# sakehl/SKA-SDP-Accelerate-gridding

Hardware: AMD Instinct MI355X
Metric: Mvis/s gridded (w-proj, 4096^2 grid) (higher is better)
Workload: dtype f64

## Files before the change

### ska-sdp-accelerate-gridding_amd/csrc/api.hip

```cpp

#include "common.h"
#include "imaging.h"

using namespace gridhip;

namespace {

int check_common(gridhip_ctx *ctx, int64_t H, int64_t Wd, const void *grid, int64_t n, const void *u,
                 const void *v, int64_t uv_stride)
{
    if (!ctx) return GRIDHIP_EINVAL;
    if (H <= 0 || Wd <= 0 || n < 0 || uv_stride < 1)
        return fail(ctx, GRIDHIP_EINVAL, "bad size (H=%lld Wd=%lld n=%lld uv_stride=%lld)", (long long)H,
                    (long long)Wd, (long long)n, (long long)uv_stride);
    if (!grid || (n > 0 && (!u || !v))) return fail(ctx, GRIDHIP_EINVAL, "null pointer");
    if (n > (int64_t)0x7fffff00) return fail(ctx, GRIDHIP_EUNSUPPORTED, "n must be < 2^31 per call");
    return GRIDHIP_OK;
}

int check_conv2(gridhip_ctx *ctx, int64_t H, int64_t Wd, const void *grid, int64_t n, const void *u, const void *v,
                int64_t uv_stride, const void *gcf, const void *vis, int64_t W, int64_t Q, int64_t gh, int64_t gw)
{
    GH_CHECK(check_common(ctx, H, Wd, grid, n, u, v, uv_stride));
    if (!gcf || (n > 0 && !vis)) return fail(ctx, GRIDHIP_EINVAL, "null pointer");
// ... 112 lines not shown
        }
    }
    if (rc == GRIDHIP_EUNSUPPORTED) {
        p->direct = true;
        return GRIDHIP_OK;
    }
    return rc;
}

int tile_kernels(gridhip_ctx *ctx, const Prep &p, const double *gcf, const double **out)
{
    ctx->last_path = p.direct ? 4 : !p.sorted ? 3 : p.g.P > 1 || p.g.fgh != p.g.gh || p.g.fgw != p.g.gw ? 2 : 1;
    ctx->last_geom[0] = p.g.ngroups;
    ctx->last_geom[1] = p.g.Tx;
    ctx->last_geom[2] = p.g.Ty;
    ctx->last_geom[3] = p.g.imoff > 0;
    *out = gcf;
    if (p.g.P == 1 && p.g.fgh == p.g.gh && p.g.fgw == p.g.gw) return GRIDHIP_OK;
    const int64_t nsl = (int64_t)p.g.W * p.g.Q * p.g.Q;
    const size_t elems = (size_t)nsl * p.g.P * p.g.gh * p.g.gw;
    GH_CHECK(ws_reserve(ctx, ctx->ktab, elems * 16));
    int blocks = (int)((elems + 255) / 256);
    if (blocks > ctx->num_cu * 16) blocks = ctx->num_cu * 16;
    hipLaunchKernelGGL(pad_kernels_kernel, dim3(blocks), dim3(256), 0, ctx->stream, p.g, nsl, (const double2 *)gcf,
                       (double2 *)ctx->ktab.ptr);
    GH_CHECK_HIP(ctx, hipGetLastError());
    *out = (const double *)ctx->ktab.ptr;
    return GRIDHIP_OK;
}

int tile_pass(gridhip_ctx *ctx, const Prep &p, const Geom &g, int64_t nrec, const double *table, const double *vis,
              const double *grid, bool degrid, bool may_keep)
{
    if (p.sorted)
        return launch_tile_grid_sorted(ctx, g, p.block, p.lds_sorted, p.nkeys, p.batch, nrec, table, vis,
                                       const_cast<double *>(grid), degrid, may_keep);
    if (degrid) return launch_tile_degrid(ctx, g, p.block, p.lds, nrec, table, grid, const_cast<double *>(vis));
    return launch_tile_grid(ctx, g, p.block, p.lds, nrec, table, vis, const_cast<double *>(grid));
}

}

extern "C" {

int gridhip_grid_dev(gridhip_ctx *ctx, int64_t H, int64_t Wd, double *grid, int64_t n, const double *u,
                     const double *v, int64_t uv_stride, const double *vis)
{
    GH_CHECK(check_common(ctx, H, Wd, grid, n, u, v, uv_stride));
    if (n > 0 && !vis) return fail(ctx, GRIDHIP_EINVAL, "null vis");
    GH_CHECK_HIP(ctx, hipSetDevice(ctx->device));
    mark(ctx, 0);
    mark(ctx, 1);
    GH_CHECK(launch_simple_grid(ctx, H, Wd, grid, n, u, v, uv_stride, vis));
    mark(ctx, 2);
    return GRIDHIP_OK;
}

int gridhip_convgrid2_dev(gridhip_ctx *ctx, int64_t H, int64_t Wd, double *grid, int64_t n, int64_t W, int64_t Q,
                          int64_t gh, int64_t gw, const double *gcf, const double *u, const double *v,
                          int64_t uv_stride, const int64_t *wbin, const double *vis)
{
    GH_CHECK(check_conv2(ctx, H, Wd, grid, n, u, v, uv_stride, gcf, vis, W, Q, gh, gw));
    GH_CHECK_HIP(ctx, hipSetDevice(ctx->device));
    Prep p;
    if (ctx->opt.variant == 1)
        p.direct = true;
// ... 122 lines not shown
```

### ska-sdp-accelerate-gridding_amd/csrc/common.h

```cpp
#pragma once
#include <hip/hip_runtime.h>
#include <stdint.h>
#include <stdio.h>
#include <string>
#include <unordered_set>
#include <utility>

#include "../../include/gridhip.h"

namespace gridhip {

struct VisRec {
    int32_t lxy;
    int32_t kslice;
    int32_t orig;
};
typedef unsigned long long RecWord;

struct Geom {
    int64_t H, Wd;
    int32_t W, Q, gh, gw;
    int32_t Tx, Ty;
    int32_t offx, offy;
    int32_t ntx, nty;
// ... 35 lines not shown
{
    return s < 0 ? x : __umulhi(x, m) >> s;
}
static inline void set_div_magic(Geom *g)
{
    div_magic(g->Tx, &g->mTx, &g->sTx);
    div_magic(g->Ty, &g->mTy, &g->sTy);
    div_magic(g->W, &g->mW, &g->sW);
    div_magic(g->P, &g->mP, &g->sP);
    div_magic(g->px, &g->mPx, &g->sPx);
}

static inline int bits_for(int64_t count)
{
    int b = 1;
    while (((int64_t)1 << b) < count) ++b;
    return b;
}
static inline void set_rec_bits(Geom *g)
{
    g->ob = bits_for(g->nvis);
    int64_t ks = g->nslices;
    if (g->per_vis && g->nvis > ks) ks = g->nvis;
    g->kb = bits_for(ks);
}
static inline bool rec_fits(const Geom &g, int limit = 64) { return g.ob + g.kb + 14 <= limit; }
__host__ __device__ __forceinline__ RecWord rec_pack(const Geom &g, int32_t lxy, int32_t kslice, int32_t orig)
{
    return (RecWord)(uint32_t)orig | (RecWord)(uint32_t)kslice << g.ob | (RecWord)((uint32_t)lxy & 0x7f) << (g.ob + g.kb) |
           (RecWord)(((uint32_t)lxy >> 16) & 0x7f) << (g.ob + g.kb + 7);
}

struct Options {
    int64_t tile = 0, block = 0, chunk = 0, wgroups = 0, variant = 0, sort = 0, dbg = 0, prepass = 0, fault_inject = 0, aw_cache = 1, aw_batch = 0, tile_x = 0, tile_y = 0, coarse_shift = 0, scatter_chunk = 0, count_unroll = 0, rec_bits = 0, wtable = 0, reserve_cus = 0, subfoot = 0, bigtile = 0, yield_cus = 0, bin_reuse = 0, list_reuse = 0;
};

struct Workspace {
    void *ptr = nullptr;
    size_t bytes = 0;
};

struct BinKey {
    Geom g;
    int64_t n, stride;
    const void *u, *v, *wbin;
    int64_t opt[5];
    const void *recs, *tables, *dig;
    uint64_t gen;
};
struct BinKeep {
    bool valid = false;
    BinKey key;
    bool pending = false;
    int backoff = 0;
    int32_t *host_flag = nullptr;
    int32_t *host_flag_dev = nullptr;
    int64_t verified = 0;
    bool verifying = false;
};
struct ListKeep {
    bool valid = false;
    uint64_t gen = 0;
    int64_t nrec = 0;
    int32_t nkeys = 0, batch = 0, ngroups = 0, ntiles = 0, Tx = 0, Ty = 0, ldw = 0, Q = 0, W = 0, P = 0;
    const void *list = nullptr, *staged = nullptr;
};
constexpr int SC_MATCH = 104, SC_VDROPPED = 105, SC_REUSED = 106, SC_GEN = 108;

struct ImagingState;

}

struct gridhip_ctx {
    int device = 0;
    hipStream_t own_stream = nullptr;
    hipStream_t stream = nullptr;
    hipEvent_t order_ev = nullptr;
    std::string err;
    gridhip::Options opt;
    gridhip::Workspace recs;
    gridhip::Workspace tables;
    gridhip::Workspace sorted;
    gridhip::Workspace recs_raw;
    gridhip::Workspace list_staged;
    gridhip::Workspace bin_digest;
    gridhip::Workspace recs_tmp;
    gridhip::Workspace blockhist;
    gridhip::Workspace ktab;
    gridhip::Workspace aw;
    int32_t *d_scalars = nullptr;
    uint64_t bin_gen = 0;
    gridhip::BinKeep keep;
    gridhip::ListKeep lists;
    int list_hold = 0;
    int64_t lists_reused = 0;
    int num_cu = 256;
    int max_lds = 160 * 1024;
    bool timing = false;
    static constexpr int EV_RING = 64;
    hipEvent_t ev[EV_RING * 3] = {};
    int64_t ev_calls = 0;
    bool ev_open = false;
    uint32_t attr_mask = 0;
    std::unordered_set<const void *> lds_raised;
    gridhip::ImagingState *img = nullptr;
    int last_path = 0;
    int last_geom[4] = {0, 0, 0, 0};
    int64_t aw_tables_built = 0;
};

namespace gridhip {

int fail(gridhip_ctx *ctx, int code, const char *fmt, ...);

#define GH_CHECK_HIP(ctx, call)                                                          \
    do {                                                                                 \
        hipError_t e__ = (call);                                                         \
        if (e__ != hipSuccess)                                                           \
            return gridhip::fail((ctx), e__ == hipErrorOutOfMemory ? GRIDHIP_ENOMEM      \
                                                                   : GRIDHIP_EHIP,       \
                                 "%s failed: %s (%s:%d)", #call, hipGetErrorString(e__), \
                                 __FILE__, __LINE__);                                    \
    } while (0)

#define GH_CHECK(expr)              \
    do {                            \
        int rc__ = (expr);          \
        if (rc__ != GRIDHIP_OK)     \
// ... 110 lines not shown
```

### ska-sdp-accelerate-gridding_amd/csrc/ctx.hip

```cpp
#include <stdarg.h>
#include <string.h>

#include <stdlib.h>

#include "common.h"
#include "imaging.h"

namespace gridhip {

int fail(gridhip_ctx *ctx, int code, const char *fmt, ...)
{
    char buf[512];
    va_list ap;
    va_start(ap, fmt);
    vsnprintf(buf, sizeof buf, fmt, ap);
    va_end(ap);
    if (ctx) ctx->err = buf;
    return code;
}

int ws_reserve(gridhip_ctx *ctx, Workspace &ws, size_t bytes)
{
    if (bytes <= ws.bytes) return GRIDHIP_OK;
    GH_CHECK_HIP(ctx, hipDeviceSynchronize());
// ... 412 lines not shown
    GH_CHECK_HIP(ctx, hipSetDevice(ctx->device));
    GH_CHECK_HIP(ctx, hipStreamSynchronize(ctx->stream));
    return GRIDHIP_OK;
}

static int64_t *opt_slot(gridhip_ctx *ctx, const char *key)
{
    if (!strcmp(key, "tile")) return &ctx->opt.tile;
    if (!strcmp(key, "tile_x")) return &ctx->opt.tile_x;
    if (!strcmp(key, "tile_y")) return &ctx->opt.tile_y;
    if (!strcmp(key, "block")) return &ctx->opt.block;
    if (!strcmp(key, "chunk")) return &ctx->opt.chunk;
    if (!strcmp(key, "wgroups")) return &ctx->opt.wgroups;
    if (!strcmp(key, "variant")) return &ctx->opt.variant;
    if (!strcmp(key, "sort")) return &ctx->opt.sort;
#ifdef GRIDHIP_TUNING
    if (!strcmp(key, "dbg")) return &ctx->opt.dbg;
#endif
    if (!strcmp(key, "prepass")) return &ctx->opt.prepass;
    if (!strcmp(key, "fault_inject")) return &ctx->opt.fault_inject;
    if (!strcmp(key, "aw_cache")) return &ctx->opt.aw_cache;
    if (!strcmp(key, "aw_batch")) return &ctx->opt.aw_batch;
    if (!strcmp(key, "coarse_shift")) return &ctx->opt.coarse_shift;
    if (!strcmp(key, "scatter_chunk")) return &ctx->opt.scatter_chunk;
    if (!strcmp(key, "count_unroll")) return &ctx->opt.count_unroll;
    if (!strcmp(key, "rec_bits")) return &ctx->opt.rec_bits;
    if (!strcmp(key, "wtable")) return &ctx->opt.wtable;
    if (!strcmp(key, "reserve_cus")) return &ctx->opt.reserve_cus;
    if (!strcmp(key, "subfoot")) return &ctx->opt.subfoot;
    if (!strcmp(key, "bigtile")) return &ctx->opt.bigtile;
    if (!strcmp(key, "yield_cus")) return &ctx->opt.yield_cus;
    if (!strcmp(key, "bin_reuse")) return &ctx->opt.bin_reuse;
    if (!strcmp(key, "list_reuse")) return &ctx->opt.list_reuse;
    if (!strcmp(key, "noise_bits")) return &ctx->img->noise_bits;
    if (!strcmp(key, "dft_slices")) return &ctx->img->dft_slices;
    if (!strcmp(key, "mosaic_cull")) return &ctx->img->mosaic_cull;
    if (!strcmp(key, "rm_stage")) return &ctx->img->rm_stage;
    return nullptr;
}

int gridhip_set_option(gridhip_ctx *ctx, const char *key, int64_t value)
{
    if (!ctx || !key) return GRIDHIP_EINVAL;
    int64_t *s = opt_slot(ctx, key);
    if (!s) return fail(ctx, GRIDHIP_EINVAL, "unknown option '%s'", key);
    if (value < 0 && s != &ctx->opt.aw_batch) return fail(ctx, GRIDHIP_EINVAL, "option '%s' must be >= 0", key);
    *s = value;
    return GRIDHIP_OK;
}

int gridhip_get_option(gridhip_ctx *ctx, const char *key, int64_t *value)
{
    if (!ctx || !key || !value) return GRIDHIP_EINVAL;
    if (!strcmp(key, "errors")) {
        GH_CHECK_HIP(ctx, hipSetDevice(ctx->device));
        int32_t h = 0;
        GH_CHECK_HIP(ctx, hipMemcpyAsync(&h, ctx->d_scalars + 2, sizeof h, hipMemcpyDeviceToHost, ctx->stream));
        GH_CHECK_HIP(ctx, hipStreamSynchronize(ctx->stream));
        *value = h;
        return GRIDHIP_OK;
    }
    {
        static const char *const names[4] = {"last_wgroups", "last_tile_x", "last_tile_y", "last_bigtile"};
        for (int i = 0; i < 4; ++i)
            if (!strcmp(key, names[i])) {
                *value = ctx->last_geom[i];
                return GRIDHIP_OK;
            }
    }
    if (!strcmp(key, "aw_tables_built")) {
        *value = ctx->aw_tables_built;
        return GRIDHIP_OK;
    }
    if (!strcmp(key, "prepass_verified")) {
        *value = ctx->keep.verified;
        return GRIDHIP_OK;
    }
    if (!strcmp(key, "prepass_reused")) {
        GH_CHECK_HIP(ctx, hipSetDevice(ctx->device));
        int32_t h = 0;
        GH_CHECK_HIP(ctx, hipMemcpyAsync(&h, ctx->d_scalars + SC_REUSED, sizeof h, hipMemcpyDeviceToHost, ctx->stream));
        GH_CHECK_HIP(ctx, hipStreamSynchronize(ctx->stream));
        *value = h;
        return GRIDHIP_OK;
    }
    if (!strcmp(key, "lists_reused")) {
        *value = ctx->lists_reused;
        return GRIDHIP_OK;
    }
    if (!strcmp(key, "last_path")) {
        *value = ctx->last_path;
        return GRIDHIP_OK;
    }
    if (!strcmp(key, "clock_khz") || !strcmp(key, "aw_clock_khz")) {
        GH_CHECK_HIP(ctx, hipSetDevice(ctx->device));
        int64_t h[4] = {0, 0, 0, 0};
        GH_CHECK_HIP(ctx, hipMemcpyAsync(h, ctx->d_scalars + (key[0] == 'a' ? 96 : 20), sizeof h, hipMemcpyDeviceToHost, ctx->stream));
        GH_CHECK_HIP(ctx, hipStreamSynchronize(ctx->stream));
        const int64_t cyc = h[2] - h[0], ticks = h[3] - h[1];
        *value = ticks > 0 && cyc > 0 ? (int64_t)((double)cyc / (double)ticks * 1e5) : 0;
        return GRIDHIP_OK;
    }
    if (!strncmp(key, "prof", 4) && key[4] >= '0' && key[4] <= '9') {
        const int slot = atoi(key + 4);
        if (slot < 0 || slot >= 32) return fail(ctx, GRIDHIP_EINVAL, "unknown option '%s'", key);
        GH_CHECK_HIP(ctx, hipSetDevice(ctx->device));
        int64_t h = 0;
        GH_CHECK_HIP(ctx, hipMemcpyAsync(&h, ctx->d_scalars + 32 + 2 * slot, sizeof h, hipMemcpyDeviceToHost,
                                         ctx->stream));
        GH_CHECK_HIP(ctx, hipStreamSynchronize(ctx->stream));
        *value = h;
        return GRIDHIP_OK;
    }
    int64_t *s = opt_slot(ctx, key);
    if (!s) return fail(ctx, GRIDHIP_EINVAL, "unknown option '%s'", key);
    *value = *s;
    return GRIDHIP_OK;
}

int gridhip_malloc(gridhip_ctx *ctx, void **dptr, int64_t bytes)
// ... 90 lines not shown
```

### ska-sdp-accelerate-gridding_amd/csrc/tile_sorted.hip

```cpp
#include "tile_common.h"

namespace gridhip {

__device__ __forceinline__ double readlane_f64(double x, int l)
{
    return __hiloint2double(__builtin_amdgcn_readlane(__double2hiint(x), l),
                            __builtin_amdgcn_readlane(__double2loint(x), l));
}

constexpr int SORTED_IM_OFF = 65528;

__device__ const int cut15[3][16] = {{0, 106, 211, 317, 422, 500, 578, 655, 733, 781, 829, 877, 926, 958, 991, 1024},
                                     {0, 108, 221, 329, 434, 513, 596, 677, 754, 800, 852, 898, 943, 969, 998, 1024},
                                     {0, 100, 202, 303, 401, 480, 562, 641, 718, 769, 824, 875, 925, 957, 992, 1024}};

struct SortedItem {
    int32_t valid, tile, grp, staged;
    int32_t v_lo;
};


template <int S, bool DEGRID, int ABL = 0, bool AW = false, bool BT = false>
__global__ void __launch_bounds__(1024, 4) tile_grid_sorted_kernel(Geom g, const RecWord *__restrict__ recs,
                                                                const int32_t *__restrict__ bin_start,
                                                                const int32_t *__restrict__ work_start,
                                                                const double2 *__restrict__ gcf,
                                                                double2 *__restrict__ vis,
                                                                double *__restrict__ grid, int nkeys, int batch,
                                                                int32_t *__restrict__ scalars,
                                                                double2 *__restrict__ sorted_vals,
                                                                uint2 *__restrict__ sorted_mo,
                                                                uint2 *__restrict__ keep_list,
                                                                int32_t *__restrict__ keep_staged, int istride,
                                                                int lists_valid)
{
    extern __shared__ double lds[];
    constexpr int S2 = S * S;
    constexpr int TAIL0 = S2 - ((S2 + 63) / 64 - 1) * 64;
    constexpr int EXTRA = DEGRID ? 0 : (TAIL0 > 32 && TAIL0 <= 34) ? TAIL0 - 32 : (S2 > 256 && TAIL0 <= 2) ? TAIL0 : 0;
    constexpr int S2E = S2 - EXTRA;
    constexpr int NSTEP_ALL = (S2E + 63) / 64;
    constexpr int TAIL = S2E - (NSTEP_ALL - 1) * 64;
    constexpr int MAXST = DEGRID ? 4 : 5;
    constexpr int FP = (NSTEP_ALL + MAXST - 1) / MAXST;
    constexpr int KST = (NSTEP_ALL + FP - 1) / FP;
    constexpr int REM = NSTEP_ALL % FP;
    constexpr int PBASE = NSTEP_ALL / FP;
    constexpr int NSTEP = KST;
    constexpr int LASTS = (REM == 0 ? KST : KST - 1) - 1;
    constexpr bool PAIR = !DEGRID && TAIL == 32;
    const int tid = threadIdx.x, nthr = blockDim.x;
    const int lane = tid & 63, wave = __builtin_amdgcn_readfirstlane(tid >> 6), nw = nthr >> 6;
    const int plane = g.lrows * g.ldw;
    const int IMO = BT ? g.imoff / 8 : SORTED_IM_OFF / 8;
    double *lre = lds, *lim = lds + IMO;
    int32_t *hist = reinterpret_cast<int32_t *>(lim + plane);
    const int hist_words = (nkeys + 1 + 3) & ~3;
    SortedItem *desc = reinterpret_cast<SortedItem *>(hist + hist_words);
    double2 *svals_wg = sorted_vals + (size_t)blockIdx.x * 2 * batch;
    uint2 *smo_wg = sorted_mo + (size_t)blockIdx.x * 2 * batch;
    int32_t *sorig_wg = reinterpret_cast<int32_t *>(sorted_vals) + (size_t)blockIdx.x * 2 * batch;

    constexpr bool STAGE_VALS = !DEGRID && AW;
    constexpr bool STAGE_ORIG = DEGRID && AW;
    const bool keeping = !AW && keep_list != nullptr;
    const bool kept = keeping && lists_valid && __builtin_amdgcn_readfirstlane(scalars[SC_MATCH]) == 1;
    const int maxcell = (g.Ty - 1) * g.ldw + g.Tx - 1;
    const bool solo = nw == 1;
    const bool is_sorter = wave == nw - 1;
    if (is_sorter && !solo && !(g.dbg & 512)) __builtin_amdgcn_s_setprio(3);
    const bool is_walker = solo || !is_sorter;
    const int nwalk = solo ? 1 : nw - 1;
    const int ncell = g.lrows * g.lcols;

    if (blockIdx.x == 0 && tid == 0) {
        long long *st = reinterpret_cast<long long *>(scalars + 20);
        st[0] = (long long)__builtin_amdgcn_s_memtime();
        st[1] = (long long)__builtin_amdgcn_s_memrealtime();
    }
    long long prof[7] = {0, 0, 0, 0, 0, 0, 0}, pt = 0;
#define GH_STAMP(i_)                        \
    if ((ABL & 16) && lane == 0) {          \
        const long long now_ = clock64();   \
        prof[i_] += now_ - pt;              \
        pt = now_;                          \
    }
    if ((ABL & 16) && lane == 0) pt = clock64();

    int32_t *queue = scalars + 4;
    int turn = 0;
    int items_left = ((int)blockIdx.x >= g.npersist) ? g.budget : 0x7fffffff;
    auto prepare = [&](int slot) {
        WorkItem w;
        int grp = 0, item = 0;
        bool have = false;
        if (items_left <= 0) turn = g.ngroups;
        --items_left;
        while (turn < g.ngroups) {
            grp = (blockIdx.x + turn) % g.ngroups;
            item = 0;
            if (lane == 0) item = atomicAdd(&queue[grp], 1);
            item = __builtin_amdgcn_readfirstlane(item);
            if (find_work_at(g, bin_start, work_start, grp, item, &w)) {
                have = true;
                break;
            }
            ++turn;
        }
        if (!have) {
            if (lane == 0) desc[slot].valid = 0;
            return;
        }
        GH_STAMP(0)
        const int first_plane = (grp * g.W + g.ngroups - 1) / g.ngroups;
        const int first_slice = first_plane * g.Q * g.Q * g.P;
        double2 *svals = svals_wg + (size_t)slot * batch;
        uint2 *smo = smo_wg + (size_t)slot * batch;
        int32_t *sorig = sorig_wg + (size_t)slot * batch;
        const int b_lo = w.v_lo;
        const int cnt = min(batch, w.v_hi - b_lo);
        int32_t *my_staged = keeping ? keep_staged + ((size_t)grp * istride + min(item, istride - 1)) : nullptr;
        if (kept) {
            if (lane == 0) {
                SortedItem d;
                d.valid = 1;
                d.tile = w.tile;
                d.grp = grp;
                d.staged = min(max(*my_staged, 0), max(cnt, 0));
                d.v_lo = b_lo;
                desc[slot] = d;
            }
            return;
        }
        if (keeping) smo = keep_list + b_lo;
        for (int i = lane; i <= nkeys; i += 64) hist[i] = 0;
        __builtin_amdgcn_fence(__ATOMIC_ACQ_REL, "wavefront");
        __builtin_amdgcn_wave_barrier();
        for (int r0 = lane; r0 < cnt; r0 += 8 * 64) {
            int key[8];
#pragma unroll
            for (int q = 0; q < 8; ++q) {
                bool off;
                key[q] = load_rec(recs, b_lo + min(r0 + q * 64, cnt - 1), g, &off).kslice - first_slice;
                if (AW) key[q] = (int)((unsigned)key[q] % (unsigned)nkeys);
                if (off) key[q] = -1;
            }
#pragma unroll
            for (int q = 0; q < 8; ++q)
                if (r0 + q * 64 < cnt && (unsigned)key[q] < (unsigned)nkeys) atomicAdd(&hist[key[q]], 1);
        }
        __builtin_amdgcn_fence(__ATOMIC_ACQ_REL, "wavefront");
        __builtin_amdgcn_wave_barrier();
        GH_STAMP(1)
        {
            const int per = (nkeys + 63) / 64;
            const int lo = min(lane * per, nkeys), hi = min(lo + per, nkeys);
            int sum = 0;
            for (int i = lo; i < hi; ++i) sum += hist[i];
            int incl = sum;
#pragma unroll
            for (int off = 1; off < 64; off <<= 1) {
                const int t = __shfl_up(incl, off, 64);
                if (lane >= off) incl += t;
            }
// ... 10 lines not shown
        int bad = 0;
        for (int r0 = lane; r0 < cnt; r0 += 8 * 64) {
            VisRec rec[8];
            double2 val[8];
            bool off[8];
#pragma unroll
            for (int q = 0; q < 8; ++q) rec[q] = load_rec(recs, b_lo + min(r0 + q * 64, cnt - 1), g, &off[q]);
            if (STAGE_VALS) {
#pragma unroll
                for (int q = 0; q < 8; ++q) val[q] = (ABL & 8) ? make_double2(1.0, (double)q) : load_nt(vis + rec[q].orig);
            }
#pragma unroll
            for (int q = 0; q < 8; ++q) {
                if (r0 + q * 64 >= cnt) break;
                int key = rec[q].kslice - first_slice;
                if (AW) key = (int)((unsigned)key % (unsigned)nkeys);
                if (off[q] || (unsigned)key >= (unsigned)nkeys) {
                    ++bad;
                    continue;
                }
                const int pos = atomicAdd(&hist[key], 1);
                if ((unsigned)pos < (unsigned)cnt) {
                    smo[pos] = make_uint2(((uint32_t)key << 16) | (uint32_t)((rec[q].lxy >> 16) * g.ldw + (rec[q].lxy & 0xffff)),
                                          (uint32_t)(AW ? rec[q].kslice : rec[q].orig));
                    if (STAGE_VALS) svals[pos] = val[q];
                    if (STAGE_ORIG) sorig[pos] = rec[q].orig;
                } else
                    ++bad;
            }
        }
        if (bad) atomicAdd(&scalars[2], bad);
        __builtin_amdgcn_fence(__ATOMIC_ACQ_REL, "wavefront");
        __builtin_amdgcn_wave_barrier();
        if (lane == 0) {
            SortedItem d;
            d.valid = 1;
            d.tile = w.tile;
            d.grp = grp;
            d.staged = min(hist[nkeys - 1], max(cnt, 0));
            d.v_lo = b_lo;
            desc[slot] = d;
            if (keeping) *my_staged = d.staged;
        }
        GH_STAMP(3)
    };

    int loff[NSTEP];
    const bool tail_ok = lane < TAIL || TAIL == 64;
#pragma unroll
    for (int s = 0; s < NSTEP; ++s) {
        int t = s * 64 + lane;
        if (FP == 1 && s == NSTEP - 1 && !tail_ok) t = PAIR ? s * 64 + lane - 32 : 0;
        loff[s] = (t / S) * g.ldw + (t % S);
    }
    const int ttail = tail_ok ? LASTS * 64 + lane : PAIR ? LASTS * 64 + lane - 32 : 0;
    const int lrow = lane / S, lcol = lane - lrow * S;

    auto walk = [&](int slot, int staged, int first_slice, int v_lo) {
        const double2 *svals = svals_wg + (size_t)slot * batch;
        const uint2 *smo = keeping ? keep_list + v_lo : smo_wg + (size_t)slot * batch;
        const int32_t *sorig = sorig_wg + (size_t)slot * batch;
        int seg_lo, seg_hi;
        if (nwalk == 15 && !DEGRID && !(g.dbg & 256)) {
            seg_lo = (int)(((int64_t)staged * cut15[g.dense][wave]) >> 10);
            seg_hi = (int)(((int64_t)staged * cut15[g.dense][wave + 1]) >> 10);
        } else {
            seg_lo = (int)(((int64_t)staged * wave) / nwalk);
            seg_hi = (int)(((int64_t)staged * (wave + 1)) / nwalk);
        }
        if (seg_lo >= seg_hi) return;
        auto load_list = [&](int b0, uint2 &mo, double2 &v, int32_t &o) {
            const int idx = max(min(b0 + lane, seg_hi - 1), seg_lo);
            mo = smo[idx];
            if (keeping) {
                const uint32_t cell = min(mo.x & 0xffffu, (uint32_t)maxcell), o_ = min(mo.y, (uint32_t)(g.nvis - 1));
                if (cell != (mo.x & 0xffffu) || o_ != mo.y) atomicAdd(&scalars[2], 1);
                mo.x = (mo.x & 0xffff0000u) | cell;
                mo.y = o_;
            }
            if (STAGE_VALS) v = svals[idx];
            if (STAGE_ORIG) o = sorig[idx];
        };
        auto load_value = [&](const uint2 &mo, double2 &v) {
            if (!DEGRID && !STAGE_VALS) v = (ABL & 8) ? make_double2(1.0, 2.0) : load_nt(vis + mo.y);
        };
        auto part_step0 = [&](int part) { return FP == 1 ? 0 : part * PBASE + min(part, REM); };
        auto part_nst = [&](int part) { return (FP == 1 || REM == 0 || part < REM) ? KST : KST - 1; };
        auto issue = [&](double2(&k)[NSTEP], int key, int len, int part) {
            key = min(max(key, 0), (AW ? g.nslices : nkeys) - 1);
            asm volatile("" : "+s"(key));
            const double2 *kp = gcf + (size_t)(first_slice + key) * S2 + 64 * part_step0(part);
            if (ABL & 4) {
#pragma unroll
                for (int s = 0; s < NSTEP; ++s) k[s] = make_double2((double)key, (double)(lane + s));
                return;
            }
            const int lofs = len > 0 ? lane : 0, lt = len > 0 ? ttail : 0;
            if (FP == 1) {
#pragma unroll
                for (int s = 0; s < NSTEP - 1; ++s) k[s] = kp[s * 64 + lofs];
                k[NSTEP - 1] = kp[lt];
            } else {
                const bool lastp = part == FP - 1, shortp = part_nst(part) < KST;
#pragma unroll
                for (int s = 0; s < NSTEP; ++s) {
                    int idx = s * 64 + lofs;
                    if (s == LASTS && lastp) idx = lt;
                    if (s == KST - 1 && shortp) idx = 0;
                    k[s] = kp[idx];
                }
            }
        };
        uint2 moN, moNN;
        double2 vN = make_double2(0.0, 0.0), vNN = make_double2(0.0, 0.0);
        int32_t oN = 0, oNN = 0;
        load_list(seg_lo, moN, vN, oN);
        load_list(seg_lo + 64, moNN, vNN, oNN);
        load_value(moN, vN);
        for (int b0 = seg_lo; b0 < seg_hi; b0 += 64) {
            const uint2 mo = moN;
            const double2 vB = vN;
            const int32_t oB = oN;
            moN = moNN;
            vN = vNN;
            oN = oNN;
            load_value(moN, vN);
            load_list(b0 + 128, moNN, vNN, oNN);
            const int bcnt = min(64, seg_hi - b0);
            const uint32_t mykey = AW ? mo.y : mo.x >> 16;
            const uint32_t prevkey = (uint32_t)__shfl_up((int)mykey, 1, 64);
            unsigned long long bits = __ballot(lane < bcnt && (lane == 0 || mykey != prevkey));
            double2 kx[EXTRA > 0 ? EXTRA : 1];
            if (EXTRA > 0) {
                const double2 *kp = gcf + (size_t)(first_slice + min((int)mykey, (AW ? g.nslices : nkeys) - 1)) * S2 + (S2 - EXTRA);
#pragma unroll
                for (int e = 0; e < EXTRA; ++e) kx[e] = (ABL & 4) ? make_double2(1.0, 2.0) : kp[e];
            }
            int lastKey = 0;
            int curKey = 0, curStart = 0, curLen = 0, curPart = FP - 1;
            auto advance = [&](int &key, int &start, int &len, int &part) {
                if (FP > 1 && curLen > 0 && curPart < FP - 1) {
                    ++curPart;
                    key = curKey;
                    start = curStart;
                    len = curLen;
                    part = curPart;
                    return;
                }
                if (bits == 0) {
                    key = lastKey;
                    start = 0;
// ... 147 lines not shown
                        const int row = lane >> 4;
                        if ((lane & 15) == 15 && i + row < len) {
                            const int32_t o = row == 0 ? oo[0] : row == 1 ? oo[1] : row == 2 ? oo[2] : oo[3];
                            if (g.P == 1 && FP == 1)
                                __builtin_nontemporal_store(dvec2_t{rr, ri}, reinterpret_cast<dvec2_t *>(vis + o));
                            else {
                                double *dst = reinterpret_cast<double *>(vis + o);
                                unsafeAtomicAdd(dst, rr);
                                unsafeAtomicAdd(dst + 1, ri);
                            }
                        }
                    }
                }
            };

            constexpr int NSETS = 3;
            double2 kS[NSETS][NSTEP];
            int keyS[NSETS], startS[NSETS], lenS[NSETS], partS[NSETS] = {0, 0, 0};
            static_assert(NSETS == 3, "initialiser of partS");
#pragma unroll
            for (int r = 0; r < NSETS - 1; ++r) {
                advance(keyS[r], startS[r], lenS[r], partS[r]);
                issue(kS[r], keyS[r], lenS[r], partS[r]);
            }
            int done = 0;
            for (;;) {
#pragma unroll
                for (int r = 0; r < NSETS; ++r) {
                    const int nx = (r + NSETS - 1) % NSETS;
                    advance(keyS[nx], startS[nx], lenS[nx], partS[nx]);
                    issue(kS[nx], keyS[nx], lenS[nx], partS[nx]);
                    asm volatile("" ::: "memory");
                    __builtin_amdgcn_sched_barrier(0);
                    process(kS[r], startS[r], lenS[r], partS[r]);
                    __builtin_amdgcn_sched_barrier(0);
                    if (FP == 1 || partS[r] == FP - 1) done += lenS[r];
                }
                if (done >= bcnt) break;
            }
            if (done > bcnt) {
#pragma unroll
                for (int r = 0; r < NSETS - 1; ++r) asm volatile("" ::"v"(kS[r][0].x), "v"(kS[r][NSTEP - 1].y));
            }
            if (EXTRA > 0 && !(ABL & 1) && lane < bcnt) {
                const int lb = (int)(mo.x & 0xffff);
#pragma unroll
                for (int e = 0; e < EXTRA; ++e) {
                    const int t = S2 - EXTRA + e;
                    double *cell = lre + (lb + (t / S) * g.ldw + (t % S));
                    __hip_atomic_fetch_add(cell, vB.x * kx[e].x - vB.y * kx[e].y, __ATOMIC_RELAXED,
                                           __HIP_MEMORY_SCOPE_WORKGROUP);
                    __hip_atomic_fetch_add(cell + IMO, vB.x * kx[e].y + vB.y * kx[e].x, __ATOMIC_RELAXED,
                                           __HIP_MEMORY_SCOPE_WORKGROUP);
                }
            }
        }
    };

    const int fl_r0 = (tid >> 1) / g.lcols, fl_c0 = (tid >> 1) - fl_r0 * g.lcols;
    const int fl_dr = (nthr >> 1) / g.lcols, fl_dc = (nthr >> 1) - fl_dr * g.lcols;

    if (is_sorter) prepare(0);
    if (!DEGRID) {
        for (int i = tid; i < plane; i += nthr) {
            lre[i] = 0.0;
            lim[i] = 0.0;
        }
    }
    __syncthreads();
    for (int cur = 0;; cur ^= 1) {
        const SortedItem d = desc[cur];
        if (!d.valid) break;
        const int first_plane = (d.grp * g.W + g.ngroups - 1) / g.ngroups;
        const int first_slice = first_plane * g.Q * g.Q * g.P;
        const int tx = d.tile % g.ntx, ty = d.tile / g.ntx;
        const int64_t ox = (int64_t)tx * g.Tx - g.offx, oy = (int64_t)ty * g.Ty - g.offy;
        if (DEGRID) {
            const double2 *gsrc = reinterpret_cast<const double2 *>(grid);
            for (int c = tid; c < ncell; c += nthr) {
                const int r_ = c / g.lcols, c_ = c - r_ * g.lcols;
                const int64_t gx = ox + c_, gy = oy + r_;
                double2 v = make_double2(0.0, 0.0);
                if (gx >= 0 && gy >= 0 && gx < g.Wd && gy < g.H) v = gsrc[gy * g.Wd + gx];
                lre[r_ * g.ldw + c_] = v.x;
                lim[r_ * g.ldw + c_] = v.y;
            }
            __syncthreads();
        }
        const long long walk_t0 = (ABL & 16) ? clock64() : 0;
        if (is_sorter && !solo) prepare(cur ^ 1);
        if (is_walker) {
            if ((ABL & 16) && wave == 0 && lane == 0) pt = clock64();
            walk(cur, d.staged, first_slice, d.v_lo);
            if ((ABL & 16) && wave == 0) GH_STAMP(4)
        }
        if (solo) prepare(cur ^ 1);
        if ((ABL & 16) && lane == 0)
            atomicAdd(reinterpret_cast<unsigned long long *>(scalars + 32) + 8 + wave, (unsigned long long)(clock64() - walk_t0));
        __syncthreads();
        if ((ABL & 16) && wave == 0) GH_STAMP(5)
        if (DEGRID) continue;

        {
            const int comp = tid & 1;
            int r_ = fl_r0, c_ = fl_c0;
            for (int e = tid; e < 2 * ncell; e += nthr) {
                const int64_t gx = ox + c_, gy = oy + r_;
                double *cell = (comp ? lim : lre) + r_ * g.ldw + c_;
                c_ += fl_dc;
                r_ += fl_dr;
                if (c_ >= g.lcols) {
                    c_ -= g.lcols;
                    ++r_;
                }
                const double val = *cell;
                if (val == 0.0) continue;
                *cell = 0.0;
                if ((ABL & 2) || gx < 0 || gy < 0 || gx >= g.Wd || gy >= g.H) continue;
                unsafeAtomicAdd(grid + 2 * (gy * g.Wd + gx) + comp, val);
            }
        }
        __syncthreads();
        if ((ABL & 16) && wave == 0) GH_STAMP(6)
    }
    if (blockIdx.x == 0 && tid == 0) {
        long long *st = reinterpret_cast<long long *>(scalars + 20);
        st[2] = (long long)__builtin_amdgcn_s_memtime();
        st[3] = (long long)__builtin_amdgcn_s_memrealtime();
    }
    if ((ABL & 16) && lane == 0 && (wave == 0 || (is_sorter && !solo))) {
        unsigned long long *out = reinterpret_cast<unsigned long long *>(scalars + 32);
        for (int i = 0; i < 7; ++i)
            if (prof[i]) atomicAdd(&out[i], (unsigned long long)prof[i]);
    }
#undef GH_STAMP
}

bool sorted_plan(const gridhip_ctx *ctx, const Geom &g, int block, int *nkeys, int *batch, size_t *lds_bytes)
{
    if (g.gh != g.gw || g.gh < 5 || g.gh > (g.per_vis ? 16 : 32)) return false;
    const int planes = (g.W + g.ngroups - 1) / g.ngroups + 1;
    const int64_t keys = g.per_vis ? 4096 : (int64_t)planes * g.Q * g.Q * g.P;
    if (keys >= 65536) return false;
    const size_t plane = (size_t)g.lrows * g.ldw * 8;
    if (plane > (size_t)(g.imoff > 0 ? g.imoff : SORTED_IM_OFF)) return false;
    const size_t tile = (size_t)(g.imoff > 0 ? g.imoff : SORTED_IM_OFF) + plane;
    const size_t hist = (size_t)((keys + 1 + 3) & ~3) * 4;
    if (tile + hist + 128 > (size_t)ctx->max_lds) return false;
    (void)block;
    int c = ctx->opt.chunk ? (int)ctx->opt.chunk : 16384;
    c = c < 64 ? 64 : c > 16384 ? 16384 : c;
    *nkeys = (int)keys;
    *batch = c;
    *lds_bytes = tile + hist + 128;
    return true;
}

int launch_tile_grid_sorted(gridhip_ctx *ctx, const Geom &g_in, int block, size_t lds_bytes, int nkeys, int batch,
                            int64_t n, const double *gcf, const double *vis, double *grid, bool degrid, bool may_keep)
{
    Geom g = g_in;
    Tables t = tables_of(ctx, g);
    const RecWord *recs = (const RecWord *)ctx->recs.ptr;
    if (g.chunk > batch) return fail(ctx, GRIDHIP_EINVAL, "sorted kernel: chunk %d exceeds its work-item capacity %d", g.chunk, batch);
    if (g.per_vis && g.imoff > 0) return fail(ctx, GRIDHIP_EUNSUPPORTED, "no big-tile form of the aw tile kernel");
    int per_cu = (int)((size_t)ctx->max_lds / lds_bytes);
    per_cu = per_cu < 1 ? 1 : per_cu > 4 ? 4 : per_cu;
    if (per_cu * block > 2048) per_cu = 2048 / block > 0 ? 2048 / block : 1;
    int cus = ctx->num_cu - (int)ctx->opt.reserve_cus;
    if (cus < g.ngroups) cus = g.ngroups;
    int nblk = cus * per_cu;
    nblk = ctx->opt.reserve_cus ? (nblk / g.ngroups) * g.ngroups : ((nblk + g.ngroups - 1) / g.ngroups) * g.ngroups;
    const int most = work_blocks(g, n);
    if (nblk > most) nblk = most > g.ngroups ? (most / g.ngroups) * g.ngroups : g.ngroups;
    g.npersist = nblk;
    g.budget = 0;
    if (ctx->opt.yield_cus > 0 && !ctx->opt.reserve_cus) {
        int k = (((int)ctx->opt.yield_cus + 31) / 32) * 32 * per_cu;
        k = (k / g.ngroups) * g.ngroups;
        if (k > 0 && nblk - k >= g.ngroups) {
            g.npersist = nblk - k;
            g.budget = 8;
            int extra = most - g.npersist;
            extra = extra > 2048 ? 2048 : extra;
            extra = (extra / g.ngroups) * g.ngroups;
            nblk = g.npersist + (extra > k ? extra : k);
        }
    }
    const dim3 gr(nblk), bl(block);
    const BinKeep &bk = ctx->keep;
    const bool keeping = may_keep && !g.per_vis && ctx->list_hold == 0 && ctx->opt.list_reuse != 1 && ctx->opt.bin_reuse != 1 && bk.valid &&
                         bk.key.gen == ctx->bin_gen && bk.key.recs == ctx->recs.ptr && bk.key.n == n && n > 0 &&
                         ctx->recs_raw.bytes >= (size_t)n * sizeof(uint2);
    const int istride = g.nrec / g.chunk + g.ntiles + 1;
    uint2 *klist = nullptr;
    int32_t *kstaged = nullptr;
    int lists_valid = 0;
    const ListKeep was = ctx->lists;
    ListKeep now;
    ctx->lists.valid = false;
    if (keeping) {
        GH_CHECK(ws_reserve(ctx, ctx->list_staged, (size_t)g.ngroups * istride * sizeof(int32_t)));
        klist = (uint2 *)ctx->recs_raw.ptr;
        kstaged = (int32_t *)ctx->list_staged.ptr;
        now.valid = true;
        now.gen = ctx->bin_gen;
        now.nrec = n;
        now.nkeys = nkeys, now.batch = batch, now.ngroups = g.ngroups, now.ntiles = g.ntiles;
        now.Tx = g.Tx, now.Ty = g.Ty, now.ldw = g.ldw, now.Q = g.Q, now.W = g.W, now.P = g.P;
        now.list = klist, now.staged = kstaged;
        lists_valid = bk.verifying && was.valid && was.gen + 1 == now.gen && was.nrec == now.nrec && was.nkeys == now.nkeys &&
                      was.batch == now.batch && was.ngroups == now.ngroups && was.ntiles == now.ntiles && was.Tx == now.Tx &&
                      was.Ty == now.Ty && was.ldw == now.ldw && was.Q == now.Q && was.W == now.W && was.P == now.P &&
                      was.list == now.list && was.staged == now.staged;
        if (lists_valid) ++ctx->lists_reused;
    }
    auto done = [&]() {
        ctx->lists = now;
        return GRIDHIP_OK;
    };
    const size_t nlist = (size_t)nblk * 2 * batch, nvals = g.per_vis ? nlist : 0;
    GH_CHECK(ws_reserve(ctx, ctx->sorted, nvals * 16 + nlist * 8));
    double2 *svals = (double2 *)ctx->sorted.ptr;
    uint2 *smo = (uint2 *)(svals + nvals);
    launch_clear(ctx, t.scalars + 4, 16, (g.dbg & 16) ? t.scalars + 32 : nullptr, (g.dbg & 16) ? 64 : 0);
#define GH_LAUNCH_(S_, D_, B_)                                                                                   \
    do {                                                                                                         \
        GH_CHECK(raise_lds(ctx, tile_grid_sorted_kernel<S_, D_, 0, false, B_>));                                 \
        hipLaunchKernelGGL((tile_grid_sorted_kernel<S_, D_, 0, false, B_>), gr, bl, lds_bytes, ctx->stream, g, recs, \
                           t.bin_start, t.work_start, (const double2 *)gcf, (double2 *)vis, grid, nkeys, batch, \
                           t.scalars, svals, smo, klist, kstaged, istride, lists_valid);                         \
    } while (0)
#define GH_LAUNCH(S_, D_)                \
    do {                                 \
        if (g.imoff > 0)                 \
            GH_LAUNCH_(S_, D_, true);    \
        else                             \
            GH_LAUNCH_(S_, D_, false);   \
    } while (0)
#define GH_LAUNCH_AW_(S_, D_)                                                                                    \
    do {                                                                                                         \
        GH_CHECK(raise_lds(ctx, tile_grid_sorted_kernel<S_, D_, 0, true>));                                      \
        hipLaunchKernelGGL((tile_grid_sorted_kernel<S_, D_, 0, true>), gr, bl, lds_bytes, ctx->stream, g, recs,  \
                           t.bin_start, t.work_start, (const double2 *)gcf, (double2 *)vis, grid, nkeys, batch, \
                           t.scalars, svals, smo, klist, kstaged, istride, lists_valid);                         \
    } while (0)
#define GH_LAUNCH_AW(S_)                 \
    do {                                 \
        if (degrid)                      \
            GH_LAUNCH_AW_(S_, true);     \
        else                             \
            GH_LAUNCH_AW_(S_, false);    \
    } while (0)
#define GH_CASE(S_)             \
    case S_:                    \
        if (g.per_vis)          \
            GH_LAUNCH_AW(S_);   \
        else if (degrid)        \
            GH_LAUNCH(S_, true); \
        else                    \
            GH_LAUNCH(S_, false); \
        break;
#define GH_BIG(S_)                                                                  \
    case S_:                                                                        \
        if (g.per_vis) return fail(ctx, GRIDHIP_EUNSUPPORTED, "aw tile kernel: support %d", g.gh); \
        if (degrid)                                                                 \
            GH_LAUNCH(S_, true);                                                    \
        else                                                                        \
            GH_LAUNCH(S_, false);                                                   \
        break;
#define GH_ABL_BT(A_)                                                                                            \
    if (g.gh == 15 && !degrid && g.imoff > 0 && g.dbg == A_) {                                                   \
        GH_CHECK(raise_lds(ctx, tile_grid_sorted_kernel<15, false, A_, false, true>));                           \
        hipLaunchKernelGGL((tile_grid_sorted_kernel<15, false, A_, false, true>), gr, bl, lds_bytes, ctx->stream, g, recs, \
                           t.bin_start, t.work_start, (const double2 *)gcf, (double2 *)vis, grid, nkeys, batch, \
                           t.scalars, svals, smo, klist, kstaged, istride, lists_valid);                         \
        GH_CHECK_HIP(ctx, hipGetLastError());                                                                    \
        return done();                                                                                           \
    }
#define GH_ABL(A_)                                                                                               \
    if (g.gh == 15 && !degrid && g.imoff == 0 && g.dbg == A_) {                                                  \
        GH_CHECK(raise_lds(ctx, tile_grid_sorted_kernel<15, false, A_>));                                        \
        hipLaunchKernelGGL((tile_grid_sorted_kernel<15, false, A_>), gr, bl, lds_bytes, ctx->stream, g, recs,    \
                           t.bin_start, t.work_start, (const double2 *)gcf, (double2 *)vis, grid, nkeys, batch, \
                           t.scalars, svals, smo, klist, kstaged, istride, lists_valid);                         \
        GH_CHECK_HIP(ctx, hipGetLastError());                                                                    \
        return done();                                                                                           \
    }
#ifdef GRIDHIP_TUNING
    GH_ABL(1) GH_ABL(2) GH_ABL(3) GH_ABL(4) GH_ABL(5) GH_ABL(7) GH_ABL(8) GH_ABL(15) GH_ABL(16) GH_ABL_BT(16)
#endif
#undef GH_ABL
#undef GH_ABL_BT
    switch (g.gh) {
        GH_CASE(5) GH_CASE(6) GH_CASE(7) GH_CASE(8) GH_CASE(9) GH_CASE(10) GH_CASE(11) GH_CASE(12) GH_CASE(13)
        GH_CASE(14) GH_CASE(15) GH_CASE(16)
        GH_BIG(17) GH_BIG(18) GH_BIG(19) GH_BIG(20) GH_BIG(21) GH_BIG(22) GH_BIG(23) GH_BIG(24) GH_BIG(25) GH_BIG(26)
        GH_BIG(27) GH_BIG(28) GH_BIG(29) GH_BIG(30) GH_BIG(31) GH_BIG(32)
        default: return fail(ctx, GRIDHIP_EUNSUPPORTED, "no sorted instantiation for support %d", g.gh);
    }
#undef GH_CASE
#undef GH_BIG
#undef GH_LAUNCH
#undef GH_LAUNCH_
#undef GH_LAUNCH_AW
#undef GH_LAUNCH_AW_
    GH_CHECK_HIP(ctx, hipGetLastError());
    return done();
}

}
```

Before: 9319.

## Prestage first walker block of next work item in LDS from sorter wave

The sorter wave now prefetches each walker's first 64 records and their visibilities for the next work item into a new LDS staging area. Walkers pick these up after the barrier, which removes the first-block global-load latency from the start of each walk. LDS is placed either in an unused gap or appended only if occupancy is unchanged. The sorter does extra loads and waits, and a new option can disable the feature. Profiling counters for walk-open latency are also added.

```diff
diff --git a/ska-sdp-accelerate-gridding_amd/csrc/api.hip b/ska-sdp-accelerate-gridding_amd/csrc/api.hip
--- a/ska-sdp-accelerate-gridding_amd/csrc/api.hip
+++ b/ska-sdp-accelerate-gridding_amd/csrc/api.hip
@@ -168,6 +168,7 @@
 int tile_pass(gridhip_ctx *ctx, const Prep &p, const Geom &g, int64_t nrec, const double *table, const double *vis,
               const double *grid, bool degrid, bool may_keep)
 {
+    ctx->last_first_stage = 0;
     if (p.sorted)
         return launch_tile_grid_sorted(ctx, g, p.block, p.lds_sorted, p.nkeys, p.batch, nrec, table, vis,
                                        const_cast<double *>(grid), degrid, may_keep);
diff --git a/ska-sdp-accelerate-gridding_amd/csrc/common.h b/ska-sdp-accelerate-gridding_amd/csrc/common.h
--- a/ska-sdp-accelerate-gridding_amd/csrc/common.h
+++ b/ska-sdp-accelerate-gridding_amd/csrc/common.h
@@ -91,7 +91,7 @@
 }
 
 struct Options {
-    int64_t tile = 0, block = 0, chunk = 0, wgroups = 0, variant = 0, sort = 0, dbg = 0, prepass = 0, fault_inject = 0, aw_cache = 1, aw_batch = 0, tile_x = 0, tile_y = 0, coarse_shift = 0, scatter_chunk = 0, count_unroll = 0, rec_bits = 0, wtable = 0, reserve_cus = 0, subfoot = 0, bigtile = 0, yield_cus = 0, bin_reuse = 0, list_reuse = 0;
+    int64_t tile = 0, block = 0, chunk = 0, wgroups = 0, variant = 0, sort = 0, dbg = 0, prepass = 0, fault_inject = 0, aw_cache = 1, aw_batch = 0, tile_x = 0, tile_y = 0, coarse_shift = 0, scatter_chunk = 0, count_unroll = 0, rec_bits = 0, wtable = 0, reserve_cus = 0, subfoot = 0, bigtile = 0, yield_cus = 0, bin_reuse = 0, list_reuse = 0, first_stage = 0;
 };
 
 struct Workspace {
@@ -153,6 +153,7 @@
     gridhip::ListKeep lists;
     int list_hold = 0;
     int64_t lists_reused = 0;
+    int last_first_stage = 0;
     int num_cu = 256;
     int max_lds = 160 * 1024;
     bool timing = false;
diff --git a/ska-sdp-accelerate-gridding_amd/csrc/ctx.hip b/ska-sdp-accelerate-gridding_amd/csrc/ctx.hip
--- a/ska-sdp-accelerate-gridding_amd/csrc/ctx.hip
+++ b/ska-sdp-accelerate-gridding_amd/csrc/ctx.hip
@@ -468,6 +468,7 @@
     if (!strcmp(key, "yield_cus")) return &ctx->opt.yield_cus;
     if (!strcmp(key, "bin_reuse")) return &ctx->opt.bin_reuse;
     if (!strcmp(key, "list_reuse")) return &ctx->opt.list_reuse;
+    if (!strcmp(key, "first_stage")) return &ctx->opt.first_stage;
     if (!strcmp(key, "noise_bits")) return &ctx->img->noise_bits;
     if (!strcmp(key, "dft_slices")) return &ctx->img->dft_slices;
     if (!strcmp(key, "mosaic_cull")) return &ctx->img->mosaic_cull;
@@ -522,6 +523,10 @@
     }
     if (!strcmp(key, "lists_reused")) {
         *value = ctx->lists_reused;
+        return GRIDHIP_OK;
+    }
+    if (!strcmp(key, "last_first_stage")) {
+        *value = ctx->last_first_stage;
         return GRIDHIP_OK;
     }
     if (!strcmp(key, "last_path")) {
diff --git a/ska-sdp-accelerate-gridding_amd/csrc/tile_sorted.hip b/ska-sdp-accelerate-gridding_amd/csrc/tile_sorted.hip
--- a/ska-sdp-accelerate-gridding_amd/csrc/tile_sorted.hip
+++ b/ska-sdp-accelerate-gridding_amd/csrc/tile_sorted.hip
@@ -32,9 +32,9 @@
                                                                 uint2 *__restrict__ sorted_mo,
                                                                 uint2 *__restrict__ keep_list,
                                                                 int32_t *__restrict__ keep_staged, int istride,
-                                                                int lists_valid)
+                                                                int lists_valid, int stage_off)
 {
-    extern __shared__ double lds[];
+    extern __shared__ __align__(16) double lds[];
     constexpr int S2 = S * S;
     constexpr int TAIL0 = S2 - ((S2 + 63) / 64 - 1) * 64;
     constexpr int EXTRA = DEGRID ? 0 : (TAIL0 > 32 && TAIL0 <= 34) ? TAIL0 - 32 : (S2 > 256 && TAIL0 <= 2) ? TAIL0 : 0;
@@ -72,6 +72,29 @@
     const bool is_walker = solo || !is_sorter;
     const int nwalk = solo ? 1 : nw - 1;
     const int ncell = g.lrows * g.lcols;
+    constexpr bool FIRST = !DEGRID && !AW;
+    const bool staging = FIRST && !solo && stage_off > 0;
+    uint2 *stage_mo = reinterpret_cast<uint2 *>(reinterpret_cast<char *>(lds) + stage_off);
+    double2 *stage_v = reinterpret_cast<double2 *>(stage_mo + nwalk * 64);
+    auto piece = [&](int staged, int w, int &lo, int &hi) {
+        if (nwalk == 15 && !DEGRID && !(g.dbg & 256)) {
+            lo = (int)(((uint32_t)staged * (uint32_t)cut15[g.dense][w]) >> 10);
+            hi = (int)(((uint32_t)staged * (uint32_t)cut15[g.dense][w + 1]) >> 10);
+        } else {
+            lo = (int)(((uint32_t)staged * (uint32_t)w) / (uint32_t)nwalk);
+            hi = (int)(((uint32_t)staged * (uint32_t)(w + 1)) / (uint32_t)nwalk);
+        }
+    };
+    auto load_block = [&](const uint2 *smo, int lo, int hi, int b0, uint2 &mo) {
+        const int idx = max(min(b0 + lane, hi - 1), lo);
+        mo = smo[idx];
+        if (keeping) {
+            const uint32_t cell = min(mo.x & 0xffffu, (uint32_t)maxcell), o_ = min(mo.y, (uint32_t)(g.nvis - 1));
+            if (cell != (mo.x & 0xffffu) || o_ != mo.y) atomicAdd(&scalars[2], 1);
+            mo.x = (mo.x & 0xffff0000u) | cell;
+            mo.y = o_;
+        }
+    };
 
     if (blockIdx.x == 0 && tid == 0) {
         long long *st = reinterpret_cast<long long *>(scalars + 20);
@@ -86,10 +109,37 @@
         pt = now_;                          \
     }
     if ((ABL & 16) && lane == 0) pt = clock64();
+    long long open_t0 = 0, open_cyc = 0;
+    int open_items = 0;
+    bool open_pending = false;
 
     int32_t *queue = scalars + 4;
     int turn = 0;
     int items_left = ((int)blockIdx.x >= g.npersist) ? g.budget : 0x7fffffff;
+    auto stage_first = [&](int staged, const uint2 *smo) {
+        if (!FIRST || !staging || staged <= 0) return;
+        constexpr int R = 4;
+        for (int w0 = 0; w0 < nwalk; w0 += R) {
+            uint2 mo[R];
+            double2 v[R];
+#pragma unroll
+            for (int q = 0; q < R; ++q) {
+                int lo, hi;
+                piece(staged, min(w0 + q, nwalk - 1), lo, hi);
+                if (lo >= hi) lo = 0, hi = 1;
+                load_block(smo, lo, hi, lo, mo[q]);
+            }
+#pragma unroll
+            for (int q = 0; q < R; ++q) v[q] = (ABL & 8) ? make_double2(1.0, 2.0) : load_nt(vis + mo[q].y);
+#pragma unroll
+            for (int q = 0; q < R; ++q) {
+                if (w0 + q < nwalk) {
+                    stage_mo[(w0 + q) * 64 + lane] = mo[q];
+                    stage_v[(w0 + q) * 64 + lane] = v[q];
+                }
+            }
+        }
+    };
     auto prepare = [&](int slot) {
         WorkItem w;
         int grp = 0, item = 0;
@@ -121,15 +171,17 @@
         const int cnt = min(batch, w.v_hi - b_lo);
         int32_t *my_staged = keeping ? keep_staged + ((size_t)grp * istride + min(item, istride - 1)) : nullptr;
         if (kept) {
+            const int staged = __builtin_amdgcn_readfirstlane(min(max(*my_staged, 0), max(cnt, 0)));
             if (lane == 0) {
                 SortedItem d;
                 d.valid = 1;
                 d.tile = w.tile;
                 d.grp = grp;
-                d.staged = min(max(*my_staged, 0), max(cnt, 0));
+                d.staged = staged;
                 d.v_lo = b_lo;
                 desc[slot] = d;
             }
+            stage_first(staged, keep_list + b_lo);
             return;
         }
         if (keeping) smo = keep_list + b_lo;
@@ -206,15 +258,20 @@
         if (bad) atomicAdd(&scalars[2], bad);
         __builtin_amdgcn_fence(__ATOMIC_ACQ_REL, "wavefront");
         __builtin_amdgcn_wave_barrier();
+        const int staged = __builtin_amdgcn_readfirstlane(min(hist[nkeys - 1], max(cnt, 0)));
         if (lane == 0) {
             SortedItem d;
             d.valid = 1;
             d.tile = w.tile;
             d.grp = grp;
-            d.staged = min(hist[nkeys - 1], max(cnt, 0));
+            d.staged = staged;
             d.v_lo = b_lo;
             desc[slot] = d;
             if (keeping) *my_staged = d.staged;
+        }
+        if (FIRST && staging) {
+            asm volatile("s_waitcnt vmcnt(0)" ::: "memory");
+            stage_first(staged, smo);
         }
         GH_STAMP(3)
     };
@@ -230,28 +287,34 @@
     const int ttail = tail_ok ? LASTS * 64 + lane : PAIR ? LASTS * 64 + lane - 32 : 0;
     const int lrow = lane / S, lcol = lane - lrow * S;
 
+    uint2 preN = make_uint2(0u, 0u), preNN = make_uint2(0u, 0u);
+    double2 prevN = make_double2(0.0, 0.0);
+    bool pre = false;
+    auto take_first = [&](int slot) {
+        pre = false;
+        preN = preNN = make_uint2(0u, 0u);
+        prevN = make_double2(0.0, 0.0);
+        if (!FIRST || !staging || !is_walker) return;
+        if (!__builtin_amdgcn_readfirstlane(desc[slot].valid)) return;
+        const int staged = __builtin_amdgcn_readfirstlane(desc[slot].staged), v_lo = __builtin_amdgcn_readfirstlane(desc[slot].v_lo);
+        int lo, hi;
+        piece(staged, wave, lo, hi);
+        if (lo >= hi) return;
+        preN = stage_mo[wave * 64 + lane];
+        prevN = stage_v[wave * 64 + lane];
+        load_block(keeping ? keep_list + v_lo : smo_wg + (size_t)slot * batch, lo, hi, lo + 64, preNN);
+        pre = true;
+    };
     auto walk = [&](int slot, int staged, int first_slice, int v_lo) {
         const double2 *svals = svals_wg + (size_t)slot * batch;
         const uint2 *smo = keeping ? keep_list + v_lo : smo_wg + (size_t)slot * batch;
         const int32_t *sorig = sorig_wg + (size_t)slot * batch;
         int seg_lo, seg_hi;
-        if (nwalk == 15 && !DEGRID && !(g.dbg & 256)) {
-            seg_lo = (int)(((int64_t)staged * cut15[g.dense][wave]) >> 10);
-            seg_hi = (int)(((int64_t)staged * cut15[g.dense][wave + 1]) >> 10);
-        } else {
-            seg_lo = (int)(((int64_t)staged * wave) / nwalk);
-            seg_hi = (int)(((int64_t)staged * (wave + 1)) / nwalk);
-        }
+        piece(staged, wave, seg_lo, seg_hi);
         if (seg_lo >= seg_hi) return;
         auto load_list = [&](int b0, uint2 &mo, double2 &v, int32_t &o) {
             const int idx = max(min(b0 + lane, seg_hi - 1), seg_lo);
-            mo = smo[idx];
-            if (keeping) {
-                const uint32_t cell = min(mo.x & 0xffffu, (uint32_t)maxcell), o_ = min(mo.y, (uint32_t)(g.nvis - 1));
-                if (cell != (mo.x & 0xffffu) || o_ != mo.y) atomicAdd(&scalars[2], 1);
-                mo.x = (mo.x & 0xffff0000u) | cell;
-                mo.y = o_;
-            }
+            load_block(smo, seg_lo, seg_hi, b0, mo);
             if (STAGE_VALS) v = svals[idx];
             if (STAGE_ORIG) o = sorig[idx];
         };
@@ -288,9 +351,15 @@
         uint2 moN, moNN;
         double2 vN = make_double2(0.0, 0.0), vNN = make_double2(0.0, 0.0);
         int32_t oN = 0, oNN = 0;
-        load_list(seg_lo, moN, vN, oN);
-        load_list(seg_lo + 64, moNN, vNN, oNN);
-        load_value(moN, vN);
+        if (FIRST && pre) {
+            moN = preN;
+            vN = prevN;
+            moNN = preNN;
+        } else {
+            load_list(seg_lo, moN, vN, oN);
+            load_list(seg_lo + 64, moNN, vNN, oNN);
+            load_value(moN, vN);
+        }
         for (int b0 = seg_lo; b0 < seg_hi; b0 += 64) {
             const uint2 mo = moN;
             const double2 vB = vN;
@@ -504,6 +573,12 @@
                     issue(kS[nx], keyS[nx], lenS[nx], partS[nx]);
                     asm volatile("" ::: "memory");
                     __builtin_amdgcn_sched_barrier(0);
+                    if ((ABL & 16) && open_pending && lenS[r] > 0) {
+                        asm volatile("" ::"v"(vB.x), "v"(vB.y), "v"(kS[r][0].x), "v"(kS[r][NSTEP - 1].y));
+                        open_cyc += clock64() - open_t0;
+                        ++open_items;
+                        open_pending = false;
+                    }
                     process(kS[r], startS[r], lenS[r], partS[r]);
                     __builtin_amdgcn_sched_barrier(0);
                     if (FP == 1 || partS[r] == FP - 1) done += lenS[r];
@@ -540,6 +615,10 @@
         }
     }
     __syncthreads();
+    if (FIRST && staging) {
+        take_first(0);
+        __syncthreads();
+    }
     for (int cur = 0;; cur ^= 1) {
         const SortedItem d = desc[cur];
         if (!d.valid) break;
@@ -563,6 +642,10 @@
         if (is_sorter && !solo) prepare(cur ^ 1);
         if (is_walker) {
             if ((ABL & 16) && wave == 0 && lane == 0) pt = clock64();
+            if ((ABL & 16) && (wave == 0 || wave == nwalk - 1)) {
+                open_t0 = walk_t0;
+                open_pending = true;
+            }
             walk(cur, d.staged, first_slice, d.v_lo);
             if ((ABL & 16) && wave == 0) GH_STAMP(4)
         }
@@ -572,6 +655,7 @@
         __syncthreads();
         if ((ABL & 16) && wave == 0) GH_STAMP(5)
         if (DEGRID) continue;
+        take_first(cur ^ 1);
 
         {
             const int comp = tid & 1;
@@ -605,7 +689,27 @@
         for (int i = 0; i < 7; ++i)
             if (prof[i]) atomicAdd(&out[i], (unsigned long long)prof[i]);
     }
+    if ((ABL & 16) && lane == 0 && !solo && (wave == 0 || wave == nwalk - 1) && open_items) {
+        unsigned long long *out = reinterpret_cast<unsigned long long *>(scalars + 32) + (wave == 0 ? 24 : 25);
+        atomicAdd(out, (unsigned long long)open_cyc);
+        atomicAdd(out + 2, (unsigned long long)open_items);
+    }
 #undef GH_STAMP
+}
+
+static size_t sorted_stage_bytes(int block) { return block >= 128 ? (size_t)(block / 64 - 1) * 64 * 24 : 0; }
+static int sorted_stage_place(const Geom &g, int block, size_t base, size_t max_lds, size_t *total)
+{
+    const size_t need = sorted_stage_bytes(block);
+    *total = base;
+    if (need == 0 || g.per_vis) return 0;
+    const size_t gap = ((size_t)g.lrows * g.ldw * 8 + 15) & ~(size_t)15;
+    if (g.imoff == 0 && gap + need <= (size_t)SORTED_IM_OFF) return (int)gap;
+    const size_t off = (base + 15) & ~(size_t)15;
+    const size_t per_cu = max_lds / base, per_cu_with = max_lds / (off + need);
+    if (off + need > max_lds || (per_cu_with < 4 ? per_cu_with : 4) != (per_cu < 4 ? per_cu : 4)) return 0;
+    *total = off + need;
+    return (int)off;
 }
 
 bool sorted_plan(const gridhip_ctx *ctx, const Geom &g, int block, int *nkeys, int *batch, size_t *lds_bytes)
@@ -619,12 +723,17 @@
     const size_t tile = (size_t)(g.imoff > 0 ? g.imoff : SORTED_IM_OFF) + plane;
     const size_t hist = (size_t)((keys + 1 + 3) & ~3) * 4;
     if (tile + hist + 128 > (size_t)ctx->max_lds) return false;
-    (void)block;
+    size_t lds = tile + hist + 128;
+    if (ctx->opt.first_stage != 1) {
+        const size_t per_cu = (size_t)ctx->max_lds / lds;
+        sorted_stage_place(g, ctx->opt.block != 0 ? block : per_cu >= 4 ? 256 : per_cu >= 2 ? 512 : 1024, lds,
+                           (size_t)ctx->max_lds, &lds);
+    }
     int c = ctx->opt.chunk ? (int)ctx->opt.chunk : 16384;
     c = c < 64 ? 64 : c > 16384 ? 16384 : c;
     *nkeys = (int)keys;
     *batch = c;
-    *lds_bytes = tile + hist + 128;
+    *lds_bytes = lds;
     return true;
 }
 
@@ -660,6 +769,14 @@
         }
     }
     const dim3 gr(nblk), bl(block);
+    int stage_off = 0;
+    if (!degrid && ctx->opt.first_stage != 1) {
+        const size_t tile = (size_t)(g.imoff > 0 ? g.imoff : SORTED_IM_OFF) + (size_t)g.lrows * g.ldw * 8;
+        size_t total;
+        const int off = sorted_stage_place(g, block, tile + (size_t)((nkeys + 1 + 3) & ~3) * 4 + 128, (size_t)ctx->max_lds, &total);
+        if (total <= lds_bytes) stage_off = off;
+    }
+    ctx->last_first_stage = stage_off > 0;
     const BinKeep &bk = ctx->keep;
     const bool keeping = may_keep && !g.per_vis && ctx->list_hold == 0 && ctx->opt.list_reuse != 1 && ctx->opt.bin_reuse != 1 && bk.valid &&
                          bk.key.gen == ctx->bin_gen && bk.key.recs == ctx->recs.ptr && bk.key.n == n && n > 0 &&
@@ -701,7 +818,7 @@
         GH_CHECK(raise_lds(ctx, tile_grid_sorted_kernel<S_, D_, 0, false, B_>));                                 \
         hipLaunchKernelGGL((tile_grid_sorted_kernel<S_, D_, 0, false, B_>), gr, bl, lds_bytes, ctx->stream, g, recs, \
                            t.bin_start, t.work_start, (const double2 *)gcf, (double2 *)vis, grid, nkeys, batch, \
-                           t.scalars, svals, smo, klist, kstaged, istride, lists_valid);                         \
+                           t.scalars, svals, smo, klist, kstaged, istride, lists_valid, stage_off);                         \
     } while (0)
 #define GH_LAUNCH(S_, D_)                \
     do {                                 \
@@ -715,7 +832,7 @@
         GH_CHECK(raise_lds(ctx, tile_grid_sorted_kernel<S_, D_, 0, true>));                                      \
         hipLaunchKernelGGL((tile_grid_sorted_kernel<S_, D_, 0, true>), gr, bl, lds_bytes, ctx->stream, g, recs,  \
                            t.bin_start, t.work_start, (const double2 *)gcf, (double2 *)vis, grid, nkeys, batch, \
-                           t.scalars, svals, smo, klist, kstaged, istride, lists_valid);                         \
+                           t.scalars, svals, smo, klist, kstaged, istride, lists_valid, stage_off);                         \
     } while (0)
 #define GH_LAUNCH_AW(S_)                 \
     do {                                 \
@@ -746,7 +863,7 @@
         GH_CHECK(raise_lds(ctx, tile_grid_sorted_kernel<15, false, A_, false, true>));                           \
         hipLaunchKernelGGL((tile_grid_sorted_kernel<15, false, A_, false, true>), gr, bl, lds_bytes, ctx->stream, g, recs, \
                            t.bin_start, t.work_start, (const double2 *)gcf, (double2 *)vis, grid, nkeys, batch, \
-                           t.scalars, svals, smo, klist, kstaged, istride, lists_valid);                         \
+                           t.scalars, svals, smo, klist, kstaged, istride, lists_valid, stage_off);                         \
         GH_CHECK_HIP(ctx, hipGetLastError());                                                                    \
         return done();                                                                                           \
     }
@@ -755,7 +872,7 @@
         GH_CHECK(raise_lds(ctx, tile_grid_sorted_kernel<15, false, A_>));                                        \
         hipLaunchKernelGGL((tile_grid_sorted_kernel<15, false, A_>), gr, bl, lds_bytes, ctx->stream, g, recs,    \
                            t.bin_start, t.work_start, (const double2 *)gcf, (double2 *)vis, grid, nkeys, batch, \
-                           t.scalars, svals, smo, klist, kstaged, istride, lists_valid);                         \
+                           t.scalars, svals, smo, klist, kstaged, istride, lists_valid, stage_off);                         \
         GH_CHECK_HIP(ctx, hipGetLastError());                                                                    \
         return done();                                                                                           \
     }
```

New measurement: 9369, median of 6. Within noise of the previous version (+0.5%).
